# alexj94/future_urban_scene_generation

Hardware: AMD Instinct MI355X
Metric: synthesised vehicle crops/sec @256x256 (higher is better)
Workload: dtype f32 tensors; conv contraction as 3 fp16 MFMA products of scaled (hi, lo) operand splits, f32 accumulate (error vs fp64 <= 1.3x the exact-f32 MFMA kernel's: observed 0.96-1.27x over 12 operand scales x 5 layers; range-guarded; exact-f32 leg in precision_legs)

## Files before the change

### future_urban_scene_generation_amd/_lib.py

```python
from __future__ import annotations

import ctypes as C
import os

_HERE = os.path.dirname(os.path.abspath(__file__))
LIB_PATH = os.environ.get("FUSG_LIB", os.path.join(_HERE, "libfusg.so"))


class FusgUnavailable(RuntimeError):
    pass


class FusgError(RuntimeError):
    pass


class Tensor(C.Structure):
    _fields_ = [("data", C.c_void_p),
                ("n", C.c_int64), ("c", C.c_int64), ("h", C.c_int64), ("w", C.c_int64),
                ("sn", C.c_int64), ("sc", C.c_int64), ("sh", C.c_int64), ("sw", C.c_int64),
                ("dtype", C.c_int32), ("_pad", C.c_int32)]


class ConvDesc(C.Structure):
# ... 24 lines not shown
                ("w3frag", C.c_void_p), ("bias3", C.c_void_p), ("wscale3", C.c_void_p),
                ("status", C.c_void_p), ("planes", C.c_int32), ("exact_f32", C.c_int32)]


class RespairDesc(C.Structure):
    _fields_ = [("x", Tensor), ("s1", Tensor), ("kb", Tensor), ("kc", Tensor),
                ("w_in", C.c_void_p), ("bias_in", C.c_void_p),
                ("wfragA", C.c_void_p), ("biasA", C.c_void_p), ("wscaleA", C.c_void_p),
                ("wfragB", C.c_void_p), ("biasB", C.c_void_p), ("wscaleB", C.c_void_p),
                ("wfrag_b", C.c_void_p), ("bias_b", C.c_void_p), ("wscale_b", C.c_void_p),
                ("wfrag_c", C.c_void_p), ("bias_c", C.c_void_p), ("wscale_c", C.c_void_p),
                ("status", C.c_void_p), ("channels", C.c_int32), ("entry", C.c_int32),
                ("cin", C.c_int32), ("kpad_in", C.c_int32), ("tap_order", C.c_int32), ("_pad", C.c_int32)]


class HgHeadDesc(C.Structure):
    _fields_ = [("y_in", Tensor), ("x", Tensor), ("score", Tensor), ("dst", Tensor),
                ("wfrag_fc", C.c_void_p), ("bias_fc", C.c_void_p), ("wscale_fc", C.c_void_p),
                ("wfrag_score", C.c_void_p), ("bias_score", C.c_void_p), ("wscale_score", C.c_void_p),
                ("wfrag_join", C.c_void_p), ("bias_join", C.c_void_p), ("wscale_join", C.c_void_p),
                ("status", C.c_void_p), ("join", C.c_int32), ("_pad", C.c_int32)]


class PackSpec(C.Structure):
    _fields_ = [(n, C.c_int32) for n in ("cout", "cin", "kh", "kw", "c0", "stride", "pad", "dil", "upsample", "cin_pad")]


class PackSizes(C.Structure):
    _fields_ = [("cout_pad", C.c_int32), ("k_pad", C.c_int32), ("c0k", C.c_int32), ("c1k", C.c_int32),
                ("wfrag_order", C.c_int32), ("_pad", C.c_int32), ("wpack_floats", C.c_int64), ("ktab_ints", C.c_int64),
                ("wpack_h_halves", C.c_int64), ("wfrag_halves", C.c_int64)]


F32, U8, I32 = 0, 1, 2
PAD_ZERO, PAD_REFLECT, PAD_REPLICATE = 0, 1, 2
PRE_NONE, PRE_RELU, PRE_ELU, PRE_AFFINE_RELU, PRE_AFFINE = 0, 1, 2, 3, 4
ACT_NONE, ACT_RELU, ACT_TANH, ACT_SIGMOID, ACT_TANH01 = 0, 1, 2, 3, 4
STORE_NORMAL, STORE_D2S, STORE_S2D = 0, 1, 2
PREC_F32, PREC_F16X3, PREC_EMU_BF16, PREC_EMU_BF16X2, PREC_BF16 = 0, 1, 2, 3, 4
MAX_FRAMES = 64
TILE_AUTO, TILE_128x128, TILE_128x64, TILE_128x32, TILE_64x64, TILE_64x128 = 0, 1, 2, 3, 4, 5

_TP = C.POINTER(Tensor)
_SIGS = {
    "fusg_conv2d": (C.c_int, [C.POINTER(ConvDesc), C.c_void_p]),
    "fusg_conv2d_plan": (C.c_int64, [C.POINTER(ConvDesc)]),
    "fusg_conv2d_route": (C.c_int, [C.POINTER(ConvDesc)]),
    "fusg_set_route_batch": (C.c_int, [C.c_int32]),
    "fusg_route_batch": (C.c_int32, []),
    "fusg_conv2d_route_order": (C.c_int, [C.POINTER(ConvDesc), C.POINTER(C.c_int32 * 4)]),
    "fusg_hg_bottleneck": (C.c_int, [C.POINTER(BneckDesc), C.c_void_p]),
    "fusg_vunet_respair": (C.c_int, [C.POINTER(RespairDesc), C.c_void_p]),
    "fusg_hg_head": (C.c_int, [C.POINTER(HgHeadDesc), C.c_void_p]),
    "fusg_conv2d_entry_nin": (C.c_int, [C.POINTER(ConvDesc), C.POINTER(ConvDesc), C.c_void_p]),
    "fusg_conv2d_entry_nin_route": (C.c_int, [C.POINTER(ConvDesc), C.POINTER(ConvDesc)]),
    "fusg_chan_stats": (C.c_int, [_TP, C.c_void_p, C.c_int32, C.c_void_p]),
    "fusg_in_finalize": (C.c_int, [_TP, C.c_void_p, C.c_int32, C.c_float, C.c_void_p, C.c_void_p, C.c_void_p]),
    "fusg_ln_finalize": (C.c_int, [_TP, C.c_void_p, C.c_int32, C.c_float, C.c_void_p, C.c_void_p, C.c_void_p,
                                   C.c_void_p, C.c_void_p]),
    "fusg_in_finalize_slots": (C.c_int, [C.c_void_p, C.c_int32, C.c_int32, C.c_int32, C.c_float, C.c_void_p, C.c_void_p, C.c_void_p]),
    "fusg_ln_finalize_slots": (C.c_int, [C.c_void_p, C.c_int32, C.c_int32, C.c_int32, C.c_float, C.c_void_p, C.c_void_p,
                                         C.c_void_p, C.c_void_p, C.c_void_p]),
    "fusg_affine_act": (C.c_int, [_TP, C.c_void_p, C.c_void_p, C.c_int64, C.c_int32, _TP, _TP, C.c_void_p]),
    "fusg_maxpool2": (C.c_int, [_TP, _TP, C.c_void_p]),
    "fusg_upsample2_add": (C.c_int, [_TP, _TP, _TP, C.c_void_p]),
    "fusg_copy4d": (C.c_int, [_TP, _TP, C.c_int32, C.c_void_p]),
    "fusg_add4d": (C.c_int, [_TP, _TP, _TP, C.c_void_p]),
    "fusg_space_to_depth2": (C.c_int, [_TP, _TP, C.c_void_p]),
    "fusg_depth_to_space2": (C.c_int, [_TP, _TP, C.c_void_p]),
    "fusg_ec_inputs": (C.c_int, [_TP, _TP, _TP, _TP, C.c_int32, C.c_void_p]),
    "fusg_hshift_sum": (C.c_int, [_TP, C.c_void_p, C.c_int32, C.c_int32, C.c_int32, C.c_int32, _TP, C.c_void_p]),
    "fusg_argmax_hw": (C.c_int, [_TP, C.c_void_p, C.c_void_p]),
    "fusg_to_image_u8": (C.c_int, [_TP, _TP, C.c_void_p]),
    "fusg_merge_u8": (C.c_int, [_TP, _TP, _TP, _TP, C.c_void_p]),
    "fusg_warp_perspective_u8": (C.c_int, [_TP, C.c_void_p, _TP, C.c_void_p]),
    "fusg_warp_perspective_indexed_u8": (C.c_int, [_TP, C.c_void_p, C.c_void_p, C.c_int32, _TP, C.c_void_p]),
# ... 49 lines not shown
    "fusg_plan_end": (C.c_int, [C.c_void_p]),
    "fusg_plan_add_dependency": (C.c_int, [C.c_void_p, C.c_void_p, C.c_void_p]),
    "fusg_plan_add_h2d": (C.c_int, [C.c_void_p, C.c_void_p, C.c_void_p, C.c_int64, C.c_int32, C.c_int64, C.c_void_p]),
    "fusg_plan_next_slot": (C.c_int, [C.c_void_p]),
    "fusg_plan_size": (C.c_int64, [C.c_void_p]),
    "fusg_plan_run": (C.c_int, [C.c_void_p]),
    "fusg_plan_streams": (C.c_int32, [C.c_void_p]),
    "fusg_plan_run_mt": (C.c_int, [C.c_void_p]),
    "fusg_plan_graph_capture": (C.c_int, [C.c_void_p, C.c_void_p, C.c_int32]),
    "fusg_plan_graph_nodes": (C.c_int64, [C.c_void_p]),
    "fusg_plan_graph_slot": (C.c_int, [C.c_void_p]),
    "fusg_plan_graph_launch": (C.c_int, [C.c_void_p, C.c_void_p]),
    "fusg_pack_conv_sizes": (C.c_int, [C.POINTER(PackSpec), C.POINTER(PackSizes)]),
    "fusg_pack_conv_weights": (C.c_int, [C.POINTER(PackSpec)] + [C.c_void_p] * 8),
    "fusg_version": (C.c_int, []),
    "fusg_last_error": (C.c_char_p, []),
    "fusg_last_conv_kernel": (C.c_int, []),
    "fusg_arch": (C.c_char_p, []),
    "fusg_sizeof_tensor": (C.c_int, []),
    "fusg_sizeof_conv_desc": (C.c_int, []),
    "fusg_sizeof_bneck_desc": (C.c_int, []),
    "fusg_sizeof_respair_desc": (C.c_int, []),
    "fusg_sizeof_hg_head_desc": (C.c_int, []),
    "fusg_prof_enable": (None, [C.c_int]),
    "fusg_prof_reset": (None, []),
    "fusg_prof_read": (C.c_int, [C.c_int, C.POINTER(C.c_double), C.POINTER(C.c_int64), C.POINTER(C.c_double)]),
}
EXPORTS = tuple(_SIGS.keys())

ROUTE_BATCH_ENV = int(os.environ.get("FUSG_ROUTE_BATCH", "0") or 0)

_lib = None


def lib():
    global _lib
    if _lib is None:
        if not os.path.exists(LIB_PATH):
            raise FusgUnavailable(
                f"{LIB_PATH} not found: build it with `python -c 'import __graft_entry__ as g; g.build()'` "
                "(hipcc --offload-arch=gfx950).  There is no CPU fallback.")
        import torch
        try:
            h = C.CDLL(LIB_PATH)
        except OSError as e:
            raise FusgUnavailable(f"cannot load {LIB_PATH}: {e}") from e
        for name, (res, args) in _SIGS.items():
            fn = getattr(h, name)
            fn.restype = res
            fn.argtypes = args
        if (h.fusg_sizeof_tensor() != C.sizeof(Tensor) or h.fusg_sizeof_conv_desc() != C.sizeof(ConvDesc)
                or h.fusg_sizeof_bneck_desc() != C.sizeof(BneckDesc)
                or h.fusg_sizeof_respair_desc() != C.sizeof(RespairDesc)
                or h.fusg_sizeof_hg_head_desc() != C.sizeof(HgHeadDesc)):
            raise FusgUnavailable("libfusg.so struct layout differs from the ctypes mirror (stale build?)")
        if ROUTE_BATCH_ENV and h.fusg_set_route_batch(ROUTE_BATCH_ENV) < 0:
            raise FusgError(f"FUSG_ROUTE_BATCH={ROUTE_BATCH_ENV}: {h.fusg_last_error().decode()}")
        _lib = h
    return _lib


def check(rc: int, what: str = "") -> None:
    if rc != 0:
        msg = lib().fusg_last_error()
        raise FusgError(f"{what}: rc={rc}: {msg.decode() if msg else ''}")
```

### future_urban_scene_generation_amd/csrc/common.h

```cpp
#pragma once
#include <hip/hip_runtime.h>
#include <functional>
#include <memory>
#include <tuple>
#include <utility>
#include <stdint.h>
#include <stdio.h>
#include <string.h>
#include "../../include/fusg.h"

namespace fusg {

void set_error(const char* fmt, ...);
void note_conv_kernel(int kind);

#define FUSG_CHECK(cond, ...)                         \
    do {                                              \
        if (!(cond)) {                                \
            fusg::set_error(__VA_ARGS__);             \
            return FUSG_ERR_INVALID;                  \
        }                                             \
    } while (0)

#define FUSG_LAUNCH_CHECK(what)                                                    \
// ... 54 lines not shown
    bool has; fusg_conv_desc d;
    explicit SavedArg(const fusg_conv_desc* p) : has(p != nullptr), d(p ? *p : fusg_conv_desc{}) {}
    const fusg_conv_desc* get() const { return has ? &d : nullptr; }
};

template <> struct SavedArg<const fusg_bneck_desc*> {
    bool has; fusg_bneck_desc d;
    explicit SavedArg(const fusg_bneck_desc* p) : has(p != nullptr), d(p ? *p : fusg_bneck_desc{}) {}
    const fusg_bneck_desc* get() const { return has ? &d : nullptr; }
};

template <> struct SavedArg<const fusg_respair_desc*> {
    bool has; fusg_respair_desc d;
    explicit SavedArg(const fusg_respair_desc* p) : has(p != nullptr), d(p ? *p : fusg_respair_desc{}) {}
    const fusg_respair_desc* get() const { return has ? &d : nullptr; }
};

template <> struct SavedArg<const fusg_hg_head_desc*> {
    bool has; fusg_hg_head_desc d;
    explicit SavedArg(const fusg_hg_head_desc* p) : has(p != nullptr), d(p ? *p : fusg_hg_head_desc{}) {}
    const fusg_hg_head_desc* get() const { return has ? &d : nullptr; }
};

template <class... A>
int plan_dispatch(int (*impl)(A..., void*), void* stream, A... a) {
    if (plan_recording()) {
        auto saved = std::make_shared<std::tuple<SavedArg<A>...>>(SavedArg<A>(a)...);
        const int32_t rb = route_batch_now();
        plan_append((hipStream_t)stream, [impl, saved, rb](hipStream_t s) {
            RouteBatchScope scope(rb);
            return std::apply([&](const SavedArg<A>&... sv) { return impl(sv.get()..., (void*)s); }, *saved);
        });
    }
    return impl(a..., stream);
}

const float* zero_line();

void prof_begin(int kind, hipStream_t s, double flops);
void prof_end(int kind, hipStream_t s);

}
```

### future_urban_scene_generation_amd/csrc/conv_kernel_small.h

```cpp
#pragma once
#include "conv_kernel_h3.h"

namespace fusg {

constexpr int SMALL_NS = 9;
constexpr int SMALL_ROWS = 32;
constexpr int SMALL_MAXPIX = 192;

struct SmallK {
    ConvK c;
    int kh, kw, pad_h, pad_w, stride;
    int nch0, nch32;
    int ntaps;
    unsigned long long tapslab;
    const _Float16* wfrag;
    int nt32;
    int nchw;
    int nimg;
    int rpi;
    int tpi;
    int wide;
    int pad_mode;
    int RIN, WIN, NPIX;
    int rpi_shift;
    unsigned m_wo, m_hw, m_win, m_rw, m_npix, m_taps, m_tpi;
    int part_off;
};

template <int PK>
__global__ __launch_bounds__(256, 1) void conv_small_h3(const SmallK sk) {
    const ConvK& p = sk.c;
    extern __shared__ __attribute__((aligned(16))) _Float16 smem_s[];
    const int t = threadIdx.x, lane = t & 63;
    const int wave = __builtin_amdgcn_readfirstlane(t >> 6);
    const int tile = blockIdx.x;
    const int mt = tile / p.NT, nt = tile - mt * p.NT;
    const int ks = blockIdx.z;
    const int hw = p.Ho * p.Wo;
    int b0, p0 = 0, oy_t = 0, ox_t = 0;
    if (sk.nimg == 1) {
        b0 = fdiv(mt, sk.m_tpi);
        p0 = (mt - b0 * sk.tpi) * SMALL_ROWS;
        oy_t = fdiv(p0, sk.m_wo);
        ox_t = sk.wide ? p0 - oy_t * p.Wo : 0;
    } else {
        b0 = mt * sk.nimg;
    }
    const int cg0 = ks * sk.nchw;
    const int nmine = min(sk.nch32 - cg0, sk.nchw);
    const int nsteps = nmine * sk.ntaps;
    const int NPIX = sk.NPIX;
    _Float16* Ah = smem_s;
    _Float16* Al = Ah + nmine * NPIX * 32;
    int* pixsrc = (int*)((char*)smem_s + sk.part_off);
    float* part = (float*)((char*)smem_s + sk.part_off);

    const _Float16* wbase = sk.wfrag + ((long)nt * 4 * 64 + lane) * 8;
    const long wchunk = (long)sk.nt32 * 4 * 64 * 8;
    const long wslab = (long)sk.nch32 * wchunk;
    struct BSet { h8 f[SMALL_NS][2][2]; };
    BSet bw;
    auto step_of = [&](int tt, int& cl, int& tap) __attribute__((always_inline)) {
        cl = fdiv(tt, sk.m_taps);
        tap = tt - cl * sk.ntaps;
    };
// ... 163 lines not shown
    if (p.ksplit > 1) {
        *(f32x4*)(p.ws + ((long)ks * p.M + m) * p.Cout_pad + n) = s;
        return;
    }
    if (n >= p.Cout) return;
    if (p.vec_epi) {
        f32x4 v;
#pragma unroll
        for (int c = 0; c < 4; ++c) v[c] = act_apply(fmaf(s[c], wsc[c], bs4[c]), p.act);
        if (p.res0) v += rv0;
        if (p.res1) v += rv1;
        *(f32x4*)(p.dst + po.d + co.d) = v;
    } else {
#pragma unroll
        for (int c = 0; c < 4; ++c) {
            if (n + c >= p.Cout) break;
            PixOff cc;
            chan_offsets(p, n + c, cc);
            epi_store(p, po, cc, p.bias[n + c], p.wscale ? p.wscale[n + c] : 1.f, s[c]);
        }
    }
}

inline size_t small_lds_bytes(int nchw, int npix) { return (size_t)2 * nchw * npix * 32 * sizeof(_Float16) + 4 * 32 * 32 * sizeof(float); }

hipError_t launch_small(const SmallK& k, dim3 grid, hipStream_t s, int pk);

}
```

### future_urban_scene_generation_amd/ops.py

```python
from __future__ import annotations

import ctypes as C
from typing import Optional, Tuple

import torch

from . import _lib as L
from .pack import ConvPlan

_DT = {torch.float32: L.F32, torch.uint8: L.U8, torch.int32: L.I32}

import os as _os
import numpy as _np


def _env_set(name: str) -> bool:
    return name in _os.environ


_PREC = {"f32": L.PREC_F32, "f16x3": L.PREC_F16X3,
         "bf16": L.PREC_BF16,
         "emu_bf16": L.PREC_EMU_BF16, "emu_bf16x2": L.PREC_EMU_BF16X2}
_EMU_BITS = {"emu_bf16": 8, "emu_bf16x2": 16}

# ... 673 lines not shown
def last_conv_kernel() -> int:
    return int(L.lib().fusg_last_conv_kernel())


_BORDER_TILES = {}


def border_tiles(h: int, w: int, device) -> torch.Tensor:
    key = (h, w, str(device))
    t = _BORDER_TILES.get(key)
    if t is None:
        ny, nx = h // 8, w // 16
        idx = [y * nx + x for y in range(ny) for x in range(nx) if y in (0, ny - 1) or x in (0, nx - 1)]
        t = torch.tensor(idx, dtype=torch.int32, device=device)
        _BORDER_TILES[key] = t
    return t


def up2_phases_ok(x: torch.Tensor, precision: Optional[str] = None) -> bool:
    b, c, h, w = x.shape
    return h >= 2 and w >= 2 and _os.environ.get("FUSG_NO_UP2_PHASES") is None


def conv_up2(exact: ConvPlan, phases, x: torch.Tensor, *, pre_op: int = L.PRE_NONE, pre=None, pre_bstride: int = 0,
             precision: Optional[str] = None, ring: Optional[dict] = None) -> torch.Tensor:
    if phases is None or not up2_phases_ok(x, precision):
        return conv(exact, x, pre_op=pre_op, pre=pre, pre_bstride=pre_bstride, precision=precision)
    b, c, h, w = x.shape
    out = nhwc_empty(b, exact.cout, 2 * h, 2 * w, x.device)
    halo = (((precision or PRECISION) in ("f16x3", "bf16") or ((precision or PRECISION) == "f32" and not _env_set("FUSG_NO_F32_HALO")))
            and c % 32 == 0 and h % 8 == 0 and w % 16 == 0 and _os.environ.get("FUSG_NO_HALO") is None)
    if isinstance(phases, ConvPlan):
        conv(phases, x, out=out, store=L.STORE_D2S, pre_op=pre_op, pre=pre, pre_bstride=pre_bstride,
             precision=precision, ksplit=1 if halo else 0)
    else:
        for ph, plan in enumerate(phases):
            conv(plan, x, out=out, out_stride=2, out_off=(ph >> 1, ph & 1), pre_op=pre_op, pre=pre,
                 pre_bstride=pre_bstride, precision=precision, ksplit=1 if halo else 0)
    if ring is not None:
        from .pack import up2_ring_launches
        for ry, rx, win, off in up2_ring_launches(h, w):
            if win[2] > 0 and win[3] > 0:
                conv(ring[(ry, rx)], x, out=out, q_window=win, out_stride=2, out_off=off, pre_op=pre_op, pre=pre,
                     pre_bstride=pre_bstride, precision=precision)
        return out
    for win in ((0, 0, 1, 2 * w), (2 * h - 1, 0, 1, 2 * w), (0, 0, 2 * h, 1), (0, 2 * w - 1, 2 * h, 1)):
        conv(exact, x, out=out, q_window=win, pre_op=pre_op, pre=pre, pre_bstride=pre_bstride, precision=precision)
    return out


def conv_transpose_phases(phases, x: torch.Tensor, *, pre_op: int = L.PRE_NONE, pre=None, pre_bstride: int = 0,
                          act: int = L.ACT_NONE, want_stats: bool = False, precision: Optional[str] = None):
    b, c, h, w = x.shape
    cout = phases[0].cout
    out = nhwc_empty(b, cout, 2 * h, 2 * w, x.device)
    n = h * w // 32
    fuse = (want_stats and act == L.ACT_NONE and (h * w) % 32 == 0 and cout % 4 == 0
            and _os.environ.get("FUSG_NO_VEC_EPI") is None)
    stats = torch.empty((b, 4 * n, cout, 2), device=x.device, dtype=torch.float32) if fuse else None
    for ph, plan in enumerate(phases):
        conv(plan, x, out=out, out_stride=2, out_off=(ph >> 1, ph & 1), q_size=(h, w), pre_op=pre_op, pre=pre,
             pre_bstride=pre_bstride, act=act, precision=precision, ksplit=1,
             stats_into=(stats, ph * n) if fuse else None)
    return (out, stats) if want_stats else out


def conv_rowsplit(plan: ConvPlan, x0: torch.Tensor, *, pre_op: int = L.PRE_NONE, pre=None, pre_bstride: int = 0,
                  act: int = L.ACT_NONE, nchw_out: bool = True) -> torch.Tensor:
# ... 456 lines not shown
```

### future_urban_scene_generation_amd/pack.py

```python
from __future__ import annotations

from dataclasses import dataclass, field
from typing import List,  Optional, Sequence, Tuple

import numpy as np
import torch

BK = 32


def _ru(x: int, m: int) -> int:
    return (x + m - 1) // m * m


@dataclass
class ConvPlan:
    wpack: torch.Tensor
    bias: torch.Tensor
    ktab: torch.Tensor
    cout: int
    cout_pad: int
    k_pad: int
    c_split: Tuple[int, ...]
    c0k: int
# ... 255 lines not shown
    for ky in range(5):
        for kx in range(5):
            a, b = UP2_ROWMAP[ry][ky], UP2_ROWMAP[rx][kx]
            wp[:, :, a, b] = wp[:, :, a, b] + w[:, :, ky, kx]
    return wp


def up2_ring_launches(h: int, w: int):
    out = []
    for ry, Y0, py in (("f", 0, 0), ("l", h - 1, 1)):
        out += [(ry, "e", (Y0, 1, 1, w - 1), (py, 0)), (ry, "o", (Y0, 0, 1, w - 1), (py, 1)),
                (ry, "f", (Y0, 0, 1, 1), (py, 0)), (ry, "l", (Y0, w - 1, 1, 1), (py, 1))]
    for rx, X0, px in (("f", 0, 0), ("l", w - 1, 1)):
        out += [("e", rx, (1, X0, h - 1, 1), (0, px)), ("o", rx, (0, X0, h - 1, 1), (1, px))]
    return out


def pack_conv_up2_ring(weight: torch.Tensor, bias: Optional[torch.Tensor]) -> dict:
    from . import _lib as L
    kinds = sorted({(ry, rx) for ry, rx, _, _ in up2_ring_launches(4, 4)})
    return {k: pack_conv(up2_border_weights(weight, *k), bias, stride=1, pad=1, pad_mode=L.PAD_REPLICATE) for k in kinds}


def pack_conv_up2_d2s(weight: torch.Tensor, bias: Optional[torch.Tensor]) -> ConvPlan:
    from . import _lib as L
    ws = torch.cat(up2_phase_weights(weight), dim=0)
    bs = None if bias is None else bias.detach().to("cpu", torch.float32).repeat(4)
    return pack_conv(ws, bs, stride=1, pad=1, pad_mode=L.PAD_REPLICATE)


def pack_conv_up2_phases(weight: torch.Tensor, bias: Optional[torch.Tensor]) -> List[ConvPlan]:
    from . import _lib as L
    return [pack_conv(wp, bias, stride=1, pad=1, pad_mode=L.PAD_REPLICATE) for wp in up2_phase_weights(weight)]


TAP_SPARSE_NEAREST, TAP_SPARSE_TRANSPOSE = 1, 2
TAP_SPARSE_AXIS = {TAP_SPARSE_NEAREST: ((0, 1), (1, 2)), TAP_SPARSE_TRANSPOSE: ((1,), (1, 2))}
UP2K3_ROWMAP = ((0, 1, 1), (1, 1, 2))
TK3_TAPS = (((1, 1),), ((2, 1), (0, 2)))


def tap_sparse_live(pattern: int) -> List[List[bool]]:
    ax = TAP_SPARSE_AXIS[pattern]
    return [[(dy in ax[ph >> 1]) and (dx in ax[ph & 1]) for dy in range(3) for dx in range(3)] for ph in range(4)]


# ... 131 lines not shown
```

### future_urban_scene_generation_amd/warp_learn/models.py

```python
from __future__ import annotations

from typing import List

import torch
import torch.nn as nn

from .. import _lib as L
from .. import ops, pack
from ..nn_base import ConvP, FusedNet, dev_vec, entry_point


class LayerNorm(nn.Module):

    def __init__(self, num_features: int, eps: float = 1e-5, affine: bool = True):
        super().__init__()
        self.num_features, self.eps, self.affine = num_features, eps, affine
        if affine:
            self.gamma = nn.Parameter(torch.Tensor(num_features).uniform_())
            self.beta = nn.Parameter(torch.zeros(num_features))


class Conv2dBlock(nn.Module):

    def __init__(self, input_dim, output_dim, kernel_size, stride, padding=0, norm="none", activation="relu",
# ... 60 lines not shown
    @staticmethod
    def _pack_block(blk: Conv2dBlock, device, upsample: int = 0):
        return pack.pack_conv(blk.conv.weight, blk.conv.bias, stride=blk.stride, pad=blk.padding,
                              pad_mode=L.PAD_REFLECT if blk.pad_type == "reflect" else L.PAD_ZERO,
                              upsample=upsample).to(device)

    def _pack_head(self, blk: Conv2dBlock, device):
        if blk.conv.cout * blk.kernel_size <= 32 and blk.pad_type == "reflect":
            return pack.pack_conv_rowsplit(blk.conv.weight, blk.conv.bias, pad=blk.padding, pad_mode=L.PAD_REFLECT).to(device)
        return self._pack_block(blk, device)

    def _pack_res(self, rbs: ResBlocks, device) -> List[tuple]:
        return [(self._pack_block(rb.model[0], device), self._pack_block(rb.model[1], device)) for rb in rbs.model]

    def _build_plans(self, device) -> dict:
        enc, dec = self.enc_content.model, self.dec.model
        nd = self.num_downs
        stem = enc[0]
        P = {"stem": pack.pack_conv(stem.conv.weight, stem.conv.bias, stride=1, pad=stem.padding, pad_mode=L.PAD_REFLECT,
                                    cin_pad=4).to(device),
             "down": [self._pack_block(enc[1 + i], device) for i in range(nd)],
             "enc_res": self._pack_res(enc[1 + nd], device),
             "dec_res": self._pack_res(dec[0], device),
             "up": [], "up_phases": [], "up_ring": [], "ln": [],
             "head": self._pack_head(dec[1 + 2 * nd], device)}
        for i in range(nd):
            blk = dec[2 + 2 * i]
            P["up"].append(self._pack_block(blk, device, upsample=1))
            ok = blk.kernel_size == 5 and blk.padding == 2 and blk.stride == 1 and blk.pad_type == "reflect"
            ok = ok and blk.conv.weight.shape[0] % 4 == 0
            P["up_phases"].append(pack.pack_conv_up2_d2s(blk.conv.weight, blk.conv.bias).to(device) if ok else None)
            P["up_ring"].append({k: v.to(device) for k, v in pack.pack_conv_up2_ring(blk.conv.weight, blk.conv.bias).items()}
                                if ok and ops._env_set("FUSG_UP2_RING9") else None)
            P["ln"].append((dev_vec(blk.norm.gamma, device), dev_vec(blk.norm.beta, device), blk.norm.eps))
        return P

    @staticmethod
    def _resblocks(plans, y: torch.Tensor) -> torch.Tensor:
        for pa, pb in plans:
            a, sa = ops.conv_in(pa, y)
            b, sb = ops.conv_in(pb, a, pre_op=L.PRE_AFFINE_RELU, pre=sa, pre_bstride=a.shape[1])
            y = ops.affine_act(b, sb[0], sb[1], L.ACT_NONE, res=y)
        return y

    def _encode(self, P, x: torch.Tensor) -> torch.Tensor:
        c, st = ops.conv_in(P["stem"], ops.as_nhwc(x, cpad=P["stem"].c0k))
        for p in P["down"]:
            c, st = ops.conv_in(p, c, pre_op=L.PRE_AFFINE_RELU, pre=st, pre_bstride=c.shape[1])
        y = ops.affine_act(c, st[0], st[1], L.ACT_RELU)
        return self._resblocks(P["enc_res"], y)

    def _decode(self, P, y: torch.Tensor) -> torch.Tensor:
        y = self._resblocks(P["dec_res"], y)
        pre_op, pre, bs = L.PRE_NONE, None, 0
        for p, ph, rg, (gamma, beta, eps) in zip(P["up"], P["up_phases"], P["up_ring"], P["ln"]):
            if ph is not None and ops.up2_phases_ok(y):
                y = ops.conv_up2(p, ph, y, pre_op=pre_op, pre=pre, pre_bstride=bs, ring=rg)
                pre = ops.layernorm_stats(y, gamma, beta, eps)
            else:
                y, pre = ops.conv_ln(p, y, gamma, beta, eps, pre_op=pre_op, pre=pre, pre_bstride=bs)
            pre_op, bs = L.PRE_AFFINE_RELU, y.shape[1]
        if P["head"].rowsplit is not None:
            return ops.conv_rowsplit(P["head"], y, pre_op=pre_op, pre=pre, pre_bstride=bs, act=L.ACT_TANH)
        return ops.conv(P["head"], y, pre_op=pre_op, pre=pre, pre_bstride=bs, act=L.ACT_TANH, nchw_out=True)

    @entry_point
    def decode(self, content: torch.Tensor) -> torch.Tensor:
        P = self._ensure(content)
        return self._decode(P, ops.as_nhwc(content))

    @entry_point
    def forward(self, image: torch.Tensor) -> torch.Tensor:
        P = self._ensure(image)
        if image.dim() != 4 or image.shape[1] != self.input_nc or image.shape[2] % 4 or image.shape[3] % 4:
            raise ValueError(f"G_Resnet expects [B,{self.input_nc},H,W] with H,W multiples of 4, got {tuple(image.shape)}")
        return self._decode(P, self._encode(P, image))


def get_icn_inputs(planes, sketch_normal, sketch_mask, central_crop, icn_w: int, icn_h: int):
    from .planes_utils import get_icn_inputs as _impl
# ... 2 lines not shown
```

### include/fusg.h

```cpp
#ifndef FUSG_H
#define FUSG_H

#include <stdint.h>

#ifdef __cplusplus
extern "C" {
#endif

#define FUSG_VERSION 118

typedef enum fusg_status {
    FUSG_OK = 0,
    FUSG_ERR_INVALID = -1,
    FUSG_ERR_LAUNCH = -2,
    FUSG_ERR_UNSUPPORTED = -3
} fusg_status;

typedef enum fusg_dtype { FUSG_F32 = 0, FUSG_U8 = 1, FUSG_I32 = 2 } fusg_dtype;

typedef struct fusg_tensor {
    void*   data;
    int64_t n, c, h, w;
    int64_t sn, sc, sh, sw;
    int32_t dtype;
// ... 111 lines not shown
    int32_t*     status;
    int32_t      channels;
    int32_t      entry;
    int32_t      cin, kpad_in;
    int32_t      tap_order;
    int32_t      _pad;
} fusg_respair_desc;
int fusg_vunet_respair(const fusg_respair_desc* d, void* stream);

int fusg_conv2d_entry_nin(const fusg_conv_desc* res, const fusg_conv_desc* nin, void* stream);
int fusg_conv2d_entry_nin_route(const fusg_conv_desc* res, const fusg_conv_desc* nin);

typedef struct fusg_hg_head_desc {
    fusg_tensor y_in, x, score, dst;
    const void*  wfrag_fc;    const float* bias_fc;    const float* wscale_fc;
    const void*  wfrag_score; const float* bias_score; const float* wscale_score;
    const void*  wfrag_join;  const float* bias_join;  const float* wscale_join;
    int32_t*     status;
    int32_t      join;
    int32_t      _pad;
} fusg_hg_head_desc;
int fusg_hg_head(const fusg_hg_head_desc* d, void* stream);

typedef struct fusg_pack_spec {
    int32_t cout, cin, kh, kw;
    int32_t c0;
    int32_t stride, pad, dil;
    int32_t upsample;
    int32_t cin_pad;
} fusg_pack_spec;
typedef struct fusg_pack_sizes {
    int32_t cout_pad, k_pad, c0k, c1k;
    int32_t wfrag_order;
    int32_t _pad;
    int64_t wpack_floats;
    int64_t ktab_ints;
    int64_t wpack_h_halves;
    int64_t wfrag_halves;
} fusg_pack_sizes;
int fusg_pack_conv_sizes(const fusg_pack_spec* spec, fusg_pack_sizes* sizes);
int fusg_pack_conv_weights(const fusg_pack_spec* spec, const float* weight, const float* bias, float* wpack, int32_t* ktab,
                           float* bias_pad, uint16_t* wpack_h, float* wscale, uint16_t* wfrag);


int fusg_chan_stats(const fusg_tensor* x, float* partial, int32_t nchunk, void* stream);
int fusg_in_finalize(const fusg_tensor* x, const float* partial, int32_t nchunk, float eps,
// ... 158 lines not shown
int        fusg_plan_add_h2d(fusg_plan* p, void* dst, const void* src, int64_t bytes, int32_t nslots, int64_t slot_stride, void* stream);
int        fusg_plan_next_slot(fusg_plan* p);
int64_t    fusg_plan_size(const fusg_plan* p);
int        fusg_plan_run(fusg_plan* p);
int32_t    fusg_plan_streams(fusg_plan* p);
int        fusg_plan_run_mt(fusg_plan* p);
int        fusg_plan_graph_capture(fusg_plan* p, void* capture_stream, int32_t slot);
int64_t    fusg_plan_graph_nodes(const fusg_plan* p);
int        fusg_plan_graph_slot(fusg_plan* p);
int        fusg_plan_graph_launch(fusg_plan* p, void* stream);


int         fusg_version(void);
const char* fusg_last_error(void);
enum { FUSG_CONV_GENERIC_F32 = 0, FUSG_CONV_GENERIC_F16X3 = 1, FUSG_CONV_HALO = 2, FUSG_CONV_HALO_S2D = 3,
       FUSG_CONV_TAPUNIT = 4, FUSG_CONV_HALO_BF16 = 5, FUSG_CONV_BNECK = 6 ,
       FUSG_CONV_POINTWISE = 7 ,
       FUSG_CONV_SMALL = 8 ,
       FUSG_CONV_HALO_F32 = 9 ,
       FUSG_CONV_TAPUNIT_F32 = 10 ,
       FUSG_CONV_TAPUNIT_BF16 = 11 ,
       FUSG_CONV_RESPAIR = 12 ,
       FUSG_CONV_HALO_ENTRY = 13 ,
       FUSG_CONV_HG_HEAD = 14  };
int         fusg_last_conv_kernel(void);
const char* fusg_arch(void);
int         fusg_sizeof_tensor(void);
int         fusg_sizeof_conv_desc(void);
int         fusg_sizeof_bneck_desc(void);
int         fusg_sizeof_respair_desc(void);
int         fusg_sizeof_hg_head_desc(void);
void fusg_prof_enable(int on);
void fusg_prof_reset(void);
int  fusg_prof_read(int kind, double* total_ms, int64_t* launches, double* flops);

#ifdef __cplusplus
}
#endif
#endif
```

Measured before the change: 1546.

## Fuse up2 border ring convs into one job-table driven kernel launch

Adds a new kernel that handles every border-ring fix-up of the 2x-upsample conv in a single launch. A per-job table picks each segment's border kind (12 pre-folded weight sets), its orientation and its run, and reuses the small-conv body. This replaces four exact-conv launches over the full top/bottom rows and left/right columns with folded-weight small tiles. The cost is extra packed weight memory, a new descriptor/ABI, and being limited to f16x3 with at most 288 channels.

```diff
diff --git a/future_urban_scene_generation_amd/_lib.py b/future_urban_scene_generation_amd/_lib.py
--- a/future_urban_scene_generation_amd/_lib.py
+++ b/future_urban_scene_generation_amd/_lib.py
@@ -70,6 +70,14 @@
                 ("status", C.c_void_p), ("join", C.c_int32), ("_pad", C.c_int32)]
 
 
+class Up2RingDesc(C.Structure):
+    _fields_ = [("src", Tensor), ("dst", Tensor),
+                ("wfrag", C.c_void_p), ("wscale", C.c_void_p), ("bias", C.c_void_p), ("jobs", C.c_void_p),
+                ("pre_scale", C.c_void_p), ("pre_shift", C.c_void_p), ("pre_bstride", C.c_int64),
+                ("status", C.c_void_p),
+                ("units", C.c_int32), ("cout", C.c_int32), ("cout_pad", C.c_int32), ("pre_op", C.c_int32)]
+
+
 class PackSpec(C.Structure):
     _fields_ = [(n, C.c_int32) for n in ("cout", "cin", "kh", "kw", "c0", "stride", "pad", "dil", "upsample", "cin_pad")]
 
@@ -100,6 +108,7 @@
     "fusg_hg_bottleneck": (C.c_int, [C.POINTER(BneckDesc), C.c_void_p]),
     "fusg_vunet_respair": (C.c_int, [C.POINTER(RespairDesc), C.c_void_p]),
     "fusg_hg_head": (C.c_int, [C.POINTER(HgHeadDesc), C.c_void_p]),
+    "fusg_up2_ring": (C.c_int, [C.POINTER(Up2RingDesc), C.c_void_p]),
     "fusg_conv2d_entry_nin": (C.c_int, [C.POINTER(ConvDesc), C.POINTER(ConvDesc), C.c_void_p]),
     "fusg_conv2d_entry_nin_route": (C.c_int, [C.POINTER(ConvDesc), C.POINTER(ConvDesc)]),
     "fusg_chan_stats": (C.c_int, [_TP, C.c_void_p, C.c_int32, C.c_void_p]),
@@ -195,6 +204,7 @@
     "fusg_sizeof_bneck_desc": (C.c_int, []),
     "fusg_sizeof_respair_desc": (C.c_int, []),
     "fusg_sizeof_hg_head_desc": (C.c_int, []),
+    "fusg_sizeof_up2_ring_desc": (C.c_int, []),
     "fusg_prof_enable": (None, [C.c_int]),
     "fusg_prof_reset": (None, []),
     "fusg_prof_read": (C.c_int, [C.c_int, C.POINTER(C.c_double), C.POINTER(C.c_int64), C.POINTER(C.c_double)]),
@@ -225,7 +235,8 @@
         if (h.fusg_sizeof_tensor() != C.sizeof(Tensor) or h.fusg_sizeof_conv_desc() != C.sizeof(ConvDesc)
                 or h.fusg_sizeof_bneck_desc() != C.sizeof(BneckDesc)
                 or h.fusg_sizeof_respair_desc() != C.sizeof(RespairDesc)
-                or h.fusg_sizeof_hg_head_desc() != C.sizeof(HgHeadDesc)):
+                or h.fusg_sizeof_hg_head_desc() != C.sizeof(HgHeadDesc)
+                or h.fusg_sizeof_up2_ring_desc() != C.sizeof(Up2RingDesc)):
             raise FusgUnavailable("libfusg.so struct layout differs from the ctypes mirror (stale build?)")
         if ROUTE_BATCH_ENV and h.fusg_set_route_batch(ROUTE_BATCH_ENV) < 0:
             raise FusgError(f"FUSG_ROUTE_BATCH={ROUTE_BATCH_ENV}: {h.fusg_last_error().decode()}")
diff --git a/future_urban_scene_generation_amd/csrc/common.h b/future_urban_scene_generation_amd/csrc/common.h
--- a/future_urban_scene_generation_amd/csrc/common.h
+++ b/future_urban_scene_generation_amd/csrc/common.h
@@ -100,6 +100,12 @@
     const fusg_hg_head_desc* get() const { return has ? &d : nullptr; }
 };
 
+template <> struct SavedArg<const fusg_up2_ring_desc*> {
+    bool has; fusg_up2_ring_desc d;
+    explicit SavedArg(const fusg_up2_ring_desc* p) : has(p != nullptr), d(p ? *p : fusg_up2_ring_desc{}) {}
+    const fusg_up2_ring_desc* get() const { return has ? &d : nullptr; }
+};
+
 template <class... A>
 int plan_dispatch(int (*impl)(A..., void*), void* stream, A... a) {
     if (plan_recording()) {
diff --git a/future_urban_scene_generation_amd/csrc/conv_kernel_small.h b/future_urban_scene_generation_amd/csrc/conv_kernel_small.h
--- a/future_urban_scene_generation_amd/csrc/conv_kernel_small.h
+++ b/future_urban_scene_generation_amd/csrc/conv_kernel_small.h
@@ -27,20 +27,22 @@
     int part_off;
 };
 
-template <int PK>
-__global__ __launch_bounds__(256, 1) void conv_small_h3(const SmallK sk) {
+template <int PK, bool GROUPED = false>
+__device__ __forceinline__ void small_body(const SmallK& sk, int mt, int nt, int ks, int gb0 = 0, int gp0 = 0) {
     const ConvK& p = sk.c;
     extern __shared__ __attribute__((aligned(16))) _Float16 smem_s[];
     const int t = threadIdx.x, lane = t & 63;
     const int wave = __builtin_amdgcn_readfirstlane(t >> 6);
-    const int tile = blockIdx.x;
-    const int mt = tile / p.NT, nt = tile - mt * p.NT;
-    const int ks = blockIdx.z;
     const int hw = p.Ho * p.Wo;
     int b0, p0 = 0, oy_t = 0, ox_t = 0;
     if (sk.nimg == 1) {
-        b0 = fdiv(mt, sk.m_tpi);
-        p0 = (mt - b0 * sk.tpi) * SMALL_ROWS;
+        if constexpr (GROUPED) {
+            b0 = gb0;
+            p0 = gp0;
+        } else {
+            b0 = fdiv(mt, sk.m_tpi);
+            p0 = (mt - b0 * sk.tpi) * SMALL_ROWS;
+        }
         oy_t = fdiv(p0, sk.m_wo);
         ox_t = sk.wide ? p0 - oy_t * p.Wo : 0;
     } else {
@@ -250,6 +252,13 @@
     }
 }
 
+template <int PK>
+__global__ __launch_bounds__(256, 1) void conv_small_h3(const SmallK sk) {
+    const int tile = blockIdx.x;
+    const int mt = tile / sk.c.NT, nt = tile - mt * sk.c.NT;
+    small_body<PK>(sk, mt, nt, blockIdx.z);
+}
+
 inline size_t small_lds_bytes(int nchw, int npix) { return (size_t)2 * nchw * npix * 32 * sizeof(_Float16) + 4 * 32 * 32 * sizeof(float); }
 
 hipError_t launch_small(const SmallK& k, dim3 grid, hipStream_t s, int pk);
diff --git a/future_urban_scene_generation_amd/csrc/conv_up2_ring.hip b/future_urban_scene_generation_amd/csrc/conv_up2_ring.hip
--- /dev/null
+++ b/future_urban_scene_generation_amd/csrc/conv_up2_ring.hip
@@ -0,0 +1,122 @@
+#include "conv_kernel_small.h"
+
+namespace fusg {
+
+constexpr int RING_KINDS = 12;
+constexpr int RING_REC = 8;
+constexpr int RING_NPIX = 3 * (SMALL_ROWS + 2);
+
+struct Up2RingK {
+    SmallK s;
+    const int* jobs;
+    long wkind;
+};
+
+constexpr unsigned ring_magic(int dv) { return dv < 2 ? 0u : (unsigned)(((1UL << 32) + (unsigned long)dv - 1) / (unsigned long)dv); }
+
+template <int PK>
+__global__ __launch_bounds__(256, 1) void conv_up2_ring_h3(const Up2RingK rk) {
+    const int4* rec = (const int4*)(rk.jobs + (long)blockIdx.z * RING_REC);
+    const int4 r0 = rec[0], r1 = rec[1];
+    const int H = rk.s.c.H, W = rk.s.c.W;
+    const int type = min(max(__builtin_amdgcn_readfirstlane(r0.x), 0), 2);
+    const int kind = min(max(__builtin_amdgcn_readfirstlane(r0.y), 0), RING_KINDS - 1);
+    const int qy0 = min(max(__builtin_amdgcn_readfirstlane(r0.z), 0), H - 1);
+    const int qx0 = min(max(__builtin_amdgcn_readfirstlane(r0.w), 0), W - 1);
+    const int nmax = type == 1 ? W - qx0 : (type == 0 ? H - qy0 : 1);
+    const int n = min(max(__builtin_amdgcn_readfirstlane(r1.x), 1), nmax);
+    const int py = __builtin_amdgcn_readfirstlane(r1.y) & 1, px = __builtin_amdgcn_readfirstlane(r1.z) & 1;
+    const int run = __builtin_amdgcn_readfirstlane(r1.w);
+    if (run < 0 || run > (n - 1) / SMALL_ROWS) return;
+
+    SmallK j = rk.s;
+    j.c.qy0 = qy0; j.c.qx0 = qx0;
+    j.c.Ho = type == 1 ? 1 : n; j.c.Wo = type == 1 ? n : 1;
+    j.c.M = j.c.B * n;
+    j.c.ooy[0] = py; j.c.oox[0] = px;
+    j.c.wscale = rk.s.c.wscale + (long)kind * rk.s.c.Cout_pad;
+    j.wfrag = rk.s.wfrag + (long)kind * rk.wkind;
+    j.wide = type == 1 ? 1 : 0;
+    j.RIN = type == 0 ? SMALL_ROWS + 2 : 3;
+    j.WIN = type == 1 ? SMALL_ROWS + 2 : 3;
+    j.NPIX = type == 2 ? 9 : RING_NPIX;
+    j.m_wo = type == 1 ? 1u : 0u;
+    j.m_win = type == 1 ? ring_magic(SMALL_ROWS + 2) : ring_magic(3);
+    j.m_rw = j.m_npix = type == 2 ? ring_magic(9) : ring_magic(RING_NPIX);
+    small_body<PK, true>(j, 0, (int)blockIdx.y, 0, (int)blockIdx.x, run * SMALL_ROWS);
+}
+
+}
+
+using namespace fusg;
+
+static bool ring_aligned16(const void* p) { return p != nullptr && (((uintptr_t)p) & 15) == 0; }
+
+static int up2_ring_impl(const fusg_up2_ring_desc* d, void* stream) {
+    hipStream_t s = (hipStream_t)stream;
+    FUSG_CHECK(d != nullptr, "up2_ring: null descriptor");
+    const fusg_tensor& x = d->src;
+    const fusg_tensor& o = d->dst;
+    FUSG_CHECK(is_nhwc(x) && x.n >= 1 && x.h >= 2 && x.w >= 2 && x.c >= 32 && x.c % 32 == 0,
+               "up2_ring: src must be NHWC-physical f32 [n, 32k, h >= 2, w >= 2]");
+    const int nch32 = (int)(x.c / 32);
+    FUSG_CHECK(small_lds_bytes(nch32, RING_NPIX) <= 144 * 1024, "up2_ring: %ld channels do not fit the staging (at most 288)", (long)x.c);
+    FUSG_CHECK(is_nhwc(o) && o.n == x.n && o.h == 2 * x.h && o.w == 2 * x.w && o.c == d->cout && o.data != x.data,
+               "up2_ring: dst must be NHWC-physical f32 [n, cout, 2h, 2w], distinct from src");
+    FUSG_CHECK(d->cout >= 4 && d->cout % 4 == 0 && d->cout_pad % 32 == 0 && d->cout <= d->cout_pad && d->cout_pad / 32 <= 65535,
+               "up2_ring: cout %d / cout_pad %d", d->cout, d->cout_pad);
+    FUSG_CHECK(o.sw % 4 == 0 && o.sh % 4 == 0 && o.sn % 4 == 0, "up2_ring: dst strides");
+    FUSG_CHECK(ring_aligned16(d->wfrag) && ring_aligned16(d->wscale) && ring_aligned16(d->bias) && ring_aligned16(d->jobs),
+               "up2_ring: wfrag, wscale, bias and jobs must be 16-byte aligned device arrays");
+    FUSG_CHECK(d->units >= 1 && d->units <= 65535, "up2_ring: %d units", d->units);
+    FUSG_CHECK(d->status != nullptr, "up2_ring: status word missing");
+    FUSG_CHECK(d->pre_op >= 0 && d->pre_op <= FUSG_PRE_AFFINE, "up2_ring: pre_op");
+    if (d->pre_op >= FUSG_PRE_AFFINE_RELU)
+        FUSG_CHECK(ring_aligned16(d->pre_scale) && ring_aligned16(d->pre_shift) && d->pre_bstride % 4 == 0,
+                   "up2_ring: affine pre-op needs 16B-aligned scale/shift");
+    FUSG_CHECK(x.n * x.h * x.w * x.sw < (1L << 40) && x.n * (x.h > x.w ? x.h : x.w) < (1L << 31) && x.h * x.w < (1L << 30), "up2_ring: extent");
+
+    Up2RingK k;
+    memset(&k, 0, sizeof(k));
+    ConvK& c = k.s.c;
+    c.src0 = c.src1 = (const float*)x.data;
+    c.bias = d->bias; c.wscale = d->wscale; c.status = d->status;
+    c.pre_scale = d->pre_scale; c.pre_shift = d->pre_shift; c.pre_bstride = d->pre_bstride;
+    c.dst = (float*)o.data; c.dsn = o.sn; c.dsc = o.sc; c.dsh = o.sh; c.dsw = o.sw;
+    c.H = c.Hv = (int)x.h; c.W = c.Wv = (int)x.w; c.Cs0 = c.Cs1 = (int)x.sw; c.C0 = (int)x.c;
+    c.K_pad = 9 * (int)x.c; c.nk = c.K_pad / BK; c.Cout = d->cout; c.Cout_pad = d->cout_pad; c.Cd = d->cout;
+    c.stride = 1; c.pad_mode = FUSG_PAD_REPLICATE; c.pre_op = d->pre_op; c.act = FUSG_ACT_NONE; c.store_mode = FUSG_STORE_NORMAL;
+    c.B = (int)x.n; c.NT = d->cout_pad / 32; c.osy = c.osx = 2;
+    c.ksplit = 1; c.steps_per_split = c.nk; c.vec_epi = 1;
+    c.zeros = zero_line();
+    if (!c.zeros) { set_error("up2_ring: cannot allocate the zero line"); return FUSG_ERR_LAUNCH; }
+    int pk = PK_NONE;
+    switch (d->pre_op) {
+        case FUSG_PRE_RELU: c.pre_relu = 1; break;
+        case FUSG_PRE_ELU: pk = PK_ELU; break;
+        case FUSG_PRE_AFFINE_RELU: pk = PK_AFFINE; c.pre_relu = 1; break;
+        case FUSG_PRE_AFFINE: pk = PK_AFFINE; break;
+        default: break;
+    }
+    SmallK& h = k.s;
+    h.kh = h.kw = 3; h.pad_h = h.pad_w = 1; h.stride = 1;
+    h.nch0 = h.nch32 = h.nchw = nch32; h.ntaps = 9;
+    for (int tp = 0; tp < 9; ++tp) h.tapslab |= (unsigned long long)tp << (4 * tp);
+    h.wfrag = (const _Float16*)d->wfrag; h.nt32 = d->cout_pad / 32;
+    h.nimg = 1; h.rpi = SMALL_ROWS; h.rpi_shift = 5; h.tpi = 1;
+    h.pad_mode = FUSG_PAD_REPLICATE;
+    h.m_taps = ring_magic(9);
+    h.part_off = (int)((size_t)2 * nch32 * RING_NPIX * 32 * sizeof(_Float16));
+    k.jobs = d->jobs;
+    k.wkind = 9L * nch32 * h.nt32 * 4 * 64 * 8;
+
+    const void* fn = pick_pk(pk, [](auto pkc) { return (const void*)conv_up2_ring_h3<decltype(pkc)::value>; });
+    prof_begin(0, s, 2.0 * (double)x.n * (4.0 * (x.h + x.w) - 4.0) * d->cout * c.K_pad);
+    const hipError_t e = launch_kernel(fn, dim3((unsigned)x.n, (unsigned)c.NT, (unsigned)d->units), small_lds_bytes(nch32, RING_NPIX), 144 * 1024, k, s);
+    prof_end(0, s);
+    if (e != hipSuccess) { set_error("up2_ring launch: %s", hipGetErrorString(e)); return FUSG_ERR_LAUNCH; }
+    note_conv_kernel(FUSG_CONV_UP2_RING);
+    return FUSG_OK;
+}
+extern "C" int fusg_up2_ring(const fusg_up2_ring_desc* d, void* stream) { return fusg::plan_dispatch(up2_ring_impl, stream, d); }
+extern "C" int fusg_sizeof_up2_ring_desc(void) { return (int)sizeof(fusg_up2_ring_desc); }
diff --git a/future_urban_scene_generation_amd/ops.py b/future_urban_scene_generation_amd/ops.py
--- a/future_urban_scene_generation_amd/ops.py
+++ b/future_urban_scene_generation_amd/ops.py
@@ -719,12 +719,51 @@
     return h >= 2 and w >= 2 and _os.environ.get("FUSG_NO_UP2_PHASES") is None
 
 
-def conv_up2(exact: ConvPlan, phases, x: torch.Tensor, *, pre_op: int = L.PRE_NONE, pre=None, pre_bstride: int = 0,
-             precision: Optional[str] = None, ring: Optional[dict] = None) -> torch.Tensor:
-    if phases is None or not up2_phases_ok(x, precision):
-        return conv(exact, x, pre_op=pre_op, pre=pre, pre_bstride=pre_bstride, precision=precision)
+_UP2_RING_JOBS = {}
+
+
+def up2_ring_jobs(h: int, w: int, device) -> torch.Tensor:
+    key = (h, w, str(device))
+    t = _UP2_RING_JOBS.get(key)
+    if t is None:
+        from .pack import up2_ring_jobs as jobs
+        t = _UP2_RING_JOBS[key] = torch.tensor(jobs(h, w), dtype=torch.int32, device=device)
+    return t
+
+
+def up2_ring1_ok(ring1, x: torch.Tensor, precision: Optional[str] = None) -> bool:
+    if ring1 is None or (precision or PRECISION) != "f16x3" or _env_set("FUSG_NO_UP2_RING1"):
+        return False
     b, c, h, w = x.shape
-    out = nhwc_empty(b, exact.cout, 2 * h, 2 * w, x.device)
+    return c % 32 == 0 and c <= 288 and c == ring1.cin and ring1.cout % 4 == 0 and h >= 2 and w >= 2 and is_nhwc(x)
+
+
+def up2_ring(ring1, x: torch.Tensor, out: torch.Tensor, *, pre_op: int = L.PRE_NONE, pre=None, pre_bstride: int = 0) -> torch.Tensor:
+    b, c, h, w = x.shape
+    dev = ring1.to(x.device).dev
+    jobs = up2_ring_jobs(h, w, x.device)
+    if RECORDER is not None:
+        RECORDER.keep.append(dev)
+        RECORDER.keep.append(jobs)
+        if pre is not None:
+            RECORDER.keep.append(pre)
+    d = L.Up2RingDesc()
+    d.src, d.dst = desc(x), desc(out)
+    d.wfrag, d.wscale, d.bias = dev["wfrag"].data_ptr(), dev["wscale"].data_ptr(), dev["bias"].data_ptr()
+    d.jobs, d.units = jobs.data_ptr(), int(jobs.shape[0])
+    if pre is not None:
+        d.pre_scale, d.pre_shift, d.pre_bstride = pre[0].data_ptr(), pre[1].data_ptr(), int(pre_bstride)
+    d.status = status_word(x.device).data_ptr()
+    d.cout, d.cout_pad, d.pre_op = ring1.cout, ring1.cout_pad, int(pre_op)
+    L.check(L.lib().fusg_up2_ring(C.byref(d), stream_ptr()), "up2_ring")
+    return out
+
+
+def up2_phase_launch(phases, x: torch.Tensor, *, pre_op: int = L.PRE_NONE, pre=None, pre_bstride: int = 0,
+                     precision: Optional[str] = None) -> torch.Tensor:
+    b, c, h, w = x.shape
+    cout = phases.cout // 4 if isinstance(phases, ConvPlan) else phases[0].cout
+    out = nhwc_empty(b, cout, 2 * h, 2 * w, x.device)
     halo = (((precision or PRECISION) in ("f16x3", "bf16") or ((precision or PRECISION) == "f32" and not _env_set("FUSG_NO_F32_HALO")))
             and c % 32 == 0 and h % 8 == 0 and w % 16 == 0 and _os.environ.get("FUSG_NO_HALO") is None)
     if isinstance(phases, ConvPlan):
@@ -734,6 +773,15 @@
         for ph, plan in enumerate(phases):
             conv(plan, x, out=out, out_stride=2, out_off=(ph >> 1, ph & 1), pre_op=pre_op, pre=pre,
                  pre_bstride=pre_bstride, precision=precision, ksplit=1 if halo else 0)
+    return out
+
+
+def conv_up2(exact: ConvPlan, phases, x: torch.Tensor, *, pre_op: int = L.PRE_NONE, pre=None, pre_bstride: int = 0,
+             precision: Optional[str] = None, ring: Optional[dict] = None, ring1=None) -> torch.Tensor:
+    if phases is None or not up2_phases_ok(x, precision):
+        return conv(exact, x, pre_op=pre_op, pre=pre, pre_bstride=pre_bstride, precision=precision)
+    b, c, h, w = x.shape
+    out = up2_phase_launch(phases, x, pre_op=pre_op, pre=pre, pre_bstride=pre_bstride, precision=precision)
     if ring is not None:
         from .pack import up2_ring_launches
         for ry, rx, win, off in up2_ring_launches(h, w):
@@ -741,6 +789,8 @@
                 conv(ring[(ry, rx)], x, out=out, q_window=win, out_stride=2, out_off=off, pre_op=pre_op, pre=pre,
                      pre_bstride=pre_bstride, precision=precision)
         return out
+    if up2_ring1_ok(ring1, x, precision):
+        return up2_ring(ring1, x, out, pre_op=pre_op, pre=pre, pre_bstride=pre_bstride)
     for win in ((0, 0, 1, 2 * w), (2 * h - 1, 0, 1, 2 * w), (0, 0, 2 * h, 1), (0, 2 * w - 1, 2 * h, 1)):
         conv(exact, x, out=out, q_window=win, pre_op=pre_op, pre=pre, pre_bstride=pre_bstride, precision=precision)
     return out
diff --git a/future_urban_scene_generation_amd/pack.py b/future_urban_scene_generation_amd/pack.py
--- a/future_urban_scene_generation_amd/pack.py
+++ b/future_urban_scene_generation_amd/pack.py
@@ -301,6 +301,54 @@
     return {k: pack_conv(up2_border_weights(weight, *k), bias, stride=1, pad=1, pad_mode=L.PAD_REPLICATE) for k in kinds}
 
 
+UP2_RING_KINDS = tuple(sorted({(ry, rx) for ry, rx, _, _ in up2_ring_launches(4, 4)}))
+
+
+def up2_ring_jobs(h: int, w: int) -> List[Tuple[int, ...]]:
+    recs = []
+    for ry, rx, (y0, x0, ny, nx), (py, px) in up2_ring_launches(h, w):
+        n = ny * nx
+        if n <= 0:
+            continue
+        assert ny == 1 or nx == 1
+        typ = 2 if n == 1 else (1 if ny == 1 else 0)
+        recs += [(typ, UP2_RING_KINDS.index((ry, rx)), y0, x0, n, py, px, run) for run in range((n + 31) // 32)]
+    return sorted(recs, key=lambda r: r[0] == 2)
+
+
+@dataclass
+class Up2RingGroup:
+    wfrag: torch.Tensor
+    wscale: torch.Tensor
+    bias: torch.Tensor
+    cin: int
+    cout: int
+    cout_pad: int
+    dev: dict = field(default_factory=dict)
+
+    def to(self, device) -> "Up2RingGroup":
+        key = str(device)
+        if self.dev.get("key") != key:
+            self.dev = {"key": key, "wfrag": self.wfrag.to(device).contiguous(), "wscale": self.wscale.to(device).contiguous(),
+                        "bias": self.bias.to(device).contiguous()}
+        return self
+
+
+def pack_conv_up2_ring_group(weight: torch.Tensor, bias: Optional[torch.Tensor]) -> Optional[Up2RingGroup]:
+    from . import _lib as L
+    frags, scales, plan = [], [], None
+    for k in UP2_RING_KINDS:
+        plan = pack_conv(up2_border_weights(weight, *k), bias, stride=1, pad=1, pad_mode=L.PAD_REPLICATE)
+        wsplit, wscale = split_f16x3(plan.wpack)
+        frag = frag_f16x3(wsplit, plan)
+        if frag is None:
+            return None
+        frags.append(frag)
+        scales.append(wscale)
+    return Up2RingGroup(wfrag=torch.stack(frags).contiguous(), wscale=torch.stack(scales).contiguous(), bias=plan.bias,
+                        cin=plan.c0k, cout=plan.cout, cout_pad=plan.cout_pad)
+
+
 def pack_conv_up2_d2s(weight: torch.Tensor, bias: Optional[torch.Tensor]) -> ConvPlan:
     from . import _lib as L
     ws = torch.cat(up2_phase_weights(weight), dim=0)
diff --git a/future_urban_scene_generation_amd/warp_learn/models.py b/future_urban_scene_generation_amd/warp_learn/models.py
--- a/future_urban_scene_generation_amd/warp_learn/models.py
+++ b/future_urban_scene_generation_amd/warp_learn/models.py
@@ -106,7 +106,7 @@
              "down": [self._pack_block(enc[1 + i], device) for i in range(nd)],
              "enc_res": self._pack_res(enc[1 + nd], device),
              "dec_res": self._pack_res(dec[0], device),
-             "up": [], "up_phases": [], "up_ring": [], "ln": [],
+             "up": [], "up_phases": [], "up_ring": [], "up_ring1": [], "ln": [],
              "head": self._pack_head(dec[1 + 2 * nd], device)}
         for i in range(nd):
             blk = dec[2 + 2 * i]
@@ -116,6 +116,8 @@
             P["up_phases"].append(pack.pack_conv_up2_d2s(blk.conv.weight, blk.conv.bias).to(device) if ok else None)
             P["up_ring"].append({k: v.to(device) for k, v in pack.pack_conv_up2_ring(blk.conv.weight, blk.conv.bias).items()}
                                 if ok and ops._env_set("FUSG_UP2_RING9") else None)
+            g = pack.pack_conv_up2_ring_group(blk.conv.weight, blk.conv.bias) if ok else None
+            P["up_ring1"].append(None if g is None else g.to(device))
             P["ln"].append((dev_vec(blk.norm.gamma, device), dev_vec(blk.norm.beta, device), blk.norm.eps))
         return P
 
@@ -137,9 +139,9 @@
     def _decode(self, P, y: torch.Tensor) -> torch.Tensor:
         y = self._resblocks(P["dec_res"], y)
         pre_op, pre, bs = L.PRE_NONE, None, 0
-        for p, ph, rg, (gamma, beta, eps) in zip(P["up"], P["up_phases"], P["up_ring"], P["ln"]):
+        for p, ph, rg, r1, (gamma, beta, eps) in zip(P["up"], P["up_phases"], P["up_ring"], P["up_ring1"], P["ln"]):
             if ph is not None and ops.up2_phases_ok(y):
-                y = ops.conv_up2(p, ph, y, pre_op=pre_op, pre=pre, pre_bstride=bs, ring=rg)
+                y = ops.conv_up2(p, ph, y, pre_op=pre_op, pre=pre, pre_bstride=bs, ring=rg, ring1=r1)
                 pre = ops.layernorm_stats(y, gamma, beta, eps)
             else:
                 y, pre = ops.conv_ln(p, y, gamma, beta, eps, pre_op=pre_op, pre=pre, pre_bstride=bs)
diff --git a/include/fusg.h b/include/fusg.h
--- a/include/fusg.h
+++ b/include/fusg.h
@@ -157,6 +157,20 @@
 } fusg_hg_head_desc;
 int fusg_hg_head(const fusg_hg_head_desc* d, void* stream);
 
+typedef struct fusg_up2_ring_desc {
+    fusg_tensor    src, dst;
+    const void*    wfrag;
+    const float*   wscale;
+    const float*   bias;
+    const int32_t* jobs;
+    const float*   pre_scale;
+    const float*   pre_shift;
+    int64_t        pre_bstride;
+    int32_t*       status;
+    int32_t        units, cout, cout_pad, pre_op;
+} fusg_up2_ring_desc;
+int fusg_up2_ring(const fusg_up2_ring_desc* d, void* stream);
+
 typedef struct fusg_pack_spec {
     int32_t cout, cin, kh, kw;
     int32_t c0;
@@ -361,7 +375,8 @@
        FUSG_CONV_TAPUNIT_BF16 = 11 ,
        FUSG_CONV_RESPAIR = 12 ,
        FUSG_CONV_HALO_ENTRY = 13 ,
-       FUSG_CONV_HG_HEAD = 14  };
+       FUSG_CONV_HG_HEAD = 14 ,
+       FUSG_CONV_UP2_RING = 15  };
 int         fusg_last_conv_kernel(void);
 const char* fusg_arch(void);
 int         fusg_sizeof_tensor(void);
@@ -369,6 +384,7 @@
 int         fusg_sizeof_bneck_desc(void);
 int         fusg_sizeof_respair_desc(void);
 int         fusg_sizeof_hg_head_desc(void);
+int         fusg_sizeof_up2_ring_desc(void);
 void fusg_prof_enable(int on);
 void fusg_prof_reset(void);
 int  fusg_prof_read(int kind, double* total_ms, int64_t* launches, double* flops);
```

New measurement: 1553 (median of 6 runs). No clear change (+0.4%).
